# kidusabe1/Imagined-Speech-Decoding

Measured on AMD Instinct MI355X. Metric: trials/sec end-to-end (filterbank+CNN fwd+bwd), higher is better.
Workload: dtype f32; 1 GPU; cfg2: 64ch x 2s@256Hz EEG, 9-band Butterworth(4) filterbank -> STFT(64/32) log band power -> Conv4Layers(576,32)+Linear(32,5) fwd+bwd, softmax-CE, AdamW; trials_per_gpu=4096, global_batch=4096, parallelism=dp1, streams=one stream

## Files before the change

imagined-speech-decoding_amd/csrc/conv.hip:

```cpp
#include "common.h"
#include <math.h>
#include <string.h>
#include <type_traits>
#include <vector>

namespace isd {

typedef float f32x4 __attribute__((ext_vector_type(4)));

constexpr int kTaps = 5;
constexpr int kCK = 32;
constexpr int kMaxZones = 64;

struct ZoneDesc {
  int cin;
  int idx_off;
  int64_t p_off;
  int64_t eff_off;
  int64_t wg_off;
};

struct bf16_t { unsigned short v; };
__device__ __forceinline__ float bf16_round(float x) {
  unsigned int u = __float_as_uint(x);
// ... 1519 lines not shown
    CF_MARK(24);
    __syncthreads();
    CF_MARK(25);
    {
      f32x4 acc[NJ][2];
#pragma unroll
      for (int j = 0; j < NJ; ++j)
#pragma unroll
        for (int gt = 0; gt < 2; ++gt) acc[j][gt] = (f32x4){0.f, 0.f, 0.f, 0.f};
      fused_conv_bf16<NJ>(w3s, gb, ttj, lane, acc);
      fused_store_bf16<NW, false>(acc, nullptr, tA, T1, TT, wave, q, jl);
    }
    CF_MARK(26);
    __syncthreads();
    CF_MARK(27);
    fused_wgrad_bf16(gb_base, tC_base, ct, ks, 4, nkb, q, jl, acc3);
    CF_MARK(28);
    fused_wgrad_x_bf16(tA_base, xt_base, wave, NW, nkb, q, jl, acc0, accb);
    CF_MARK(29);
  }
  {
    float* s4 = a.part4 + ((int64_t)blockIdx.x * 4 + ks) * a.slab1 + (int64_t)z * F * F * kTaps;
    float* s3 = a.part3 + ((int64_t)blockIdx.x * 4 + ks) * a.slab1 + (int64_t)z * F * F * kTaps;
    float* s0 = a.part0 + ((int64_t)blockIdx.x * NW + wave) * a.slab0 + zd.wg_off;
#pragma unroll
    for (int gt = 0; gt < 2; ++gt)
#pragma unroll
      for (int r = 0; r < 4; ++r) {
        const int g = gt * 16 + 4 * q + r, c = ct * 16 + jl;
#pragma unroll
        for (int k = 0; k < kTaps; ++k) {
          s4[((int64_t)g * F + c) * kTaps + k] = acc4[gt][k][r];
          s3[((int64_t)g * F + c) * kTaps + k] = acc3[gt][k][r];
          if (jl < cz) s0[((int64_t)g * cin1 + jl) * kTaps + k] = acc0[gt][k][r];
        }
        if (jl < kTaps) s0[((int64_t)g * cin1 + cz) * kTaps + jl] = jl == 0 ? accb[gt][r] : 0.f;
      }
  }
}

struct TailArgs {
  const void* a2;
  void* g2;
  const float* w3;
  const float* w4;
  const float* w3t;
  const float* w4t;
  const float* fc_w;
  const float* fc_b;
  const void* labels;
  float* logits;
  int64_t* pred;
  float* part;
  int64_t items;
  int T1, n_cls, label_bytes, train, slab;
  float grad_scale;
};

template <int NI>
__device__ __forceinline__ void tail_conv(const float* __restrict__ wl, const float* const (&in)[NI], int T1, int q,
                                          int jl, f32x4 (&acc)[NI][2]) {
  struct Frag {
    float af[kTaps][2];
    float bf[NI][kTaps];
  };
  bool ok[kTaps];
  int off[kTaps];
#pragma unroll
  for (int k = 0; k < kTaps; ++k) {
    const int idx = jl + k - 2;
    ok[k] = idx >= 0 && idx < T1;
    off[k] = ok[k] ? idx : 0;
  }
  auto load = [&](int cg, Frag& f) {
#pragma unroll
    for (int k = 0; k < kTaps; ++k) {
      f.af[k][0] = wl[((cg * kTaps + k) * 2 + 0) * 64];
      f.af[k][1] = wl[((cg * kTaps + k) * 2 + 1) * 64];
#pragma unroll
      for (int i = 0; i < NI; ++i) {
        const float v = in[i][(cg * 4 + q) * T1 + off[k]];
        f.bf[i][k] = ok[k] ? v : 0.f;
      }
    }
  };
  auto mma = [&](const Frag& f) {
#pragma unroll
    for (int k = 0; k < kTaps; ++k)
#pragma unroll
      for (int i = 0; i < NI; ++i) {
        acc[i][0] = __builtin_amdgcn_mfma_f32_16x16x4f32(f.af[k][0], f.bf[i][k], acc[i][0], 0, 0, 0);
        acc[i][1] = __builtin_amdgcn_mfma_f32_16x16x4f32(f.af[k][1], f.bf[i][k], acc[i][1], 0, 0, 0);
      }
  };
  Frag f0, f1;
  load(0, f0);
#pragma unroll 1
  for (int cg = 0; cg < 8; cg += 2) {
    load(cg + 1, f1);
    mma(f0);
    if (cg + 2 < 8) load(cg + 2, f0);
    mma(f1);
  }
}

template <int NI>
__device__ __forceinline__ void tail_wgrad(const float* const (&G)[NI], const float* const (&In)[NI], int T1, int q,
                                           int jl, f32x4 (&acc)[2][2][kTaps]) {
#pragma unroll 1
  for (int s = 0; s < 4; ++s) {
    const int t = s * 4 + q;
    const bool okA = t < T1;
    const int tc = okA ? t : 0;
    float a[NI][2], b[NI][2][kTaps];
#pragma unroll
    for (int i = 0; i < NI; ++i) {
#pragma unroll
      for (int gt = 0; gt < 2; ++gt) {
        const float v = G[i][(gt * 16 + jl) * T1 + tc];
        a[i][gt] = okA ? v : 0.f;
      }
#pragma unroll
      for (int ct = 0; ct < 2; ++ct)
#pragma unroll
        for (int k = 0; k < kTaps; ++k) {
          const int idx = t + k - 2;
          const bool in = okA && idx >= 0 && idx < T1;
          const float v = In[i][(ct * 16 + jl) * T1 + (in ? idx : 0)];
          b[i][ct][k] = in ? v : 0.f;
        }
    }
#pragma unroll
    for (int i = 0; i < NI; ++i)
#pragma unroll
      for (int gt = 0; gt < 2; ++gt)
#pragma unroll
        for (int ct = 0; ct < 2; ++ct)
#pragma unroll
          for (int k = 0; k < kTaps; ++k)
            acc[gt][ct][k] = __builtin_amdgcn_mfma_f32_16x16x4f32(a[i][gt], b[i][ct][k], acc[gt][ct][k], 0, 0, 0);
  }
}

template <bool BF = false>
__device__ __forceinline__ void tail_store_tile(const f32x4 (&acc)[2], float* __restrict__ tile, int T1, int q, int jl) {
  if (jl < T1) {
#pragma unroll
    for (int gt = 0; gt < 2; ++gt)
#pragma unroll
      for (int r = 0; r < 4; ++r) tile[(gt * 16 + 4 * q + r) * T1 + jl] = BF ? bf16_round(acc[gt][r]) : acc[gt][r];
  }
}

constexpr int kTailMaxCls = 16;
constexpr int kTailNI = 1;

constexpr int kTailCombV = 43;
constexpr int kTailCombCopy = kTailCombV * 64 * 4;
template <int NW, int NC, typename WF>
__device__ __forceinline__ void tail_combine_store(float* __restrict__ smem, int wave, int lane, WF&& W,
                                                   const float (&accfc)[kTailMaxCls * 32 / 64], float accb,
                                                   float loss_acc, float* __restrict__ slab, int slab_len, int n_cls) {
  constexpr int F = 32;
  __syncthreads();
  f32x4* mine = reinterpret_cast<f32x4*>(smem + (wave % NC) * kTailCombCopy) + lane;
  constexpr int n_phase = (NW + NC - 1) / NC;
#pragma unroll
  for (int ph = 0; ph < n_phase; ++ph) {
    if (wave / NC == ph) {
      auto put = [&](int v, f32x4 x) {
        if (ph) {
          const f32x4 o = mine[v * 64];
          x[0] += o[0]; x[1] += o[1]; x[2] += o[2]; x[3] += o[3];
        }
        mine[v * 64] = x;
      };
#pragma unroll
      for (int layer = 0; layer < 2; ++layer)
#pragma unroll
        for (int gt = 0; gt < 2; ++gt)
#pragma unroll
          for (int ct = 0; ct < 2; ++ct)
#pragma unroll
            for (int k = 0; k < kTaps; ++k) put(((layer * 2 + gt) * 2 + ct) * kTaps + k, W(layer, gt, ct, k));
      put(40, (f32x4){accfc[0], accfc[1], accfc[2], accfc[3]});
      put(41, (f32x4){accfc[4], accfc[5], accfc[6], accfc[7]});
      put(42, (f32x4){accb, loss_acc, 0.f, 0.f});
    }
    __syncthreads();
  }
  constexpr int n_copy = NW < NC ? NW : NC;
  const int n34 = 2 * F * F * kTaps, o_b = n34 + n_cls * F, o_loss = o_b + n_cls;
  for (int e = threadIdx.x; e < slab_len; e += NW * 64) {
    int src;
    if (e < n34) {
      const int layer = e >= F * F * kTaps, w = e - layer * F * F * kTaps;
      const int g = w / (F * kTaps), rem = w - g * (F * kTaps), c = rem / kTaps, k = rem - c * kTaps;
      const int v = ((layer * 2 + (g >> 4)) * 2 + (c >> 4)) * kTaps + k;
      src = (v * 64 + ((g & 15) >> 2) * 16 + (c & 15)) * 4 + (g & 3);
    } else if (e < o_b) {
      const int f = e - n34, j = f >> 6;
      src = ((40 + (j >> 2)) * 64 + (f & 63)) * 4 + (j & 3);
    } else if (e < o_loss) {
      src = (42 * 64 + (e - o_b)) * 4;
    } else {
      src = (42 * 64) * 4 + 1;
    }
    float v = smem[src];
#pragma unroll
    for (int c = 1; c < n_copy; ++c) v += smem[c * kTailCombCopy + src];
    slab[e] = v;
  }
}

template <int NW, bool BF>
__global__ __launch_bounds__(NW * 64) void featcnn_tail_kernel(TailArgs a) {
  extern __shared__ __attribute__((aligned(16))) float smem[];
  constexpr int F = 32, NI = kTailNI, WF = 8 * kTaps * 2 * 64;
  const int lane = threadIdx.x & 63, wave = threadIdx.x >> 6, q = lane >> 4, jl = lane & 15;
  const int T1 = a.T1, n_cls = a.n_cls;
  const int tile = F * T1, tpad = (tile + 3) & ~3;
  float* w3s = smem;
  float* w4s = w3s + WF;
  float* w3ts = w4s + WF;
  float* w4ts = w3ts + WF;
  float* fcs = w4ts + WF;
  float* priv = fcs + kTailMaxCls * (F + 1) + wave * NI * (4 * tpad + 64);
  float *tA2[NI], *tA3[NI], *tG[NI], *tH[NI], *featL[NI], *logL[NI];
#pragma unroll
  for (int i = 0; i < NI; ++i) {
    float* base = priv + i * (4 * tpad + 64);
    tA2[i] = base;
    tA3[i] = base + tpad;
    tG[i] = base + 2 * tpad;
    tH[i] = base + 3 * tpad;
    featL[i] = base + 4 * tpad;
    logL[i] = featL[i] + 32;
  }
  for (int e = threadIdx.x; e < WF / 4; e += NW * 64) {
    reinterpret_cast<float4*>(w3s)[e] = reinterpret_cast<const float4*>(a.w3)[e];
    reinterpret_cast<float4*>(w4s)[e] = reinterpret_cast<const float4*>(a.w4)[e];
    if (a.train) {
      reinterpret_cast<float4*>(w3ts)[e] = reinterpret_cast<const float4*>(a.w3t)[e];
      reinterpret_cast<float4*>(w4ts)[e] = reinterpret_cast<const float4*>(a.w4t)[e];
    }
  }
  for (int e = threadIdx.x; e < n_cls * F; e += NW * 64) fcs[e] = a.fc_w[e];
  for (int e = threadIdx.x; e < n_cls; e += NW * 64) fcs[n_cls * F + e] = a.fc_b[e];
  __syncthreads();

  f32x4 accW4[2][2][kTaps], accW3[2][2][kTaps];
#pragma unroll
  for (int g = 0; g < 2; ++g)
#pragma unroll
    for (int c = 0; c < 2; ++c)
#pragma unroll
      for (int k = 0; k < kTaps; ++k) {
        accW4[g][c][k] = (f32x4){0.f, 0.f, 0.f, 0.f};
        accW3[g][c][k] = (f32x4){0.f, 0.f, 0.f, 0.f};
      }
  float accfc[kTailMaxCls * F / 64], accb = 0.f, loss_acc = 0.f;
#pragma unroll
  for (int i = 0; i < kTailMaxCls * F / 64; ++i) accfc[i] = 0.f;
  const int n4 = tile >> 2;
  const float inv_t = 1.f / (float)T1;
  const int64_t stride = (int64_t)gridDim.x * NW * NI;

  for (int64_t first = ((int64_t)blockIdx.x * NW + wave) * NI; first < a.items; first += stride) {
    int64_t item[NI];
    bool live[NI];
#pragma unroll
    for (int i = 0; i < NI; ++i) {
      live[i] = first + i < a.items;
      item[i] = live[i] ? first + i : first;
      if constexpr (BF) {
        if (lane < 4 * T1) {
          const uint4 w = reinterpret_cast<const uint4*>((const unsigned short*)a.a2 + item[i] * tile)[lane];
          const int t = lane >> 2, g0 = (lane & 3) * 8;
          float* d = tA2[i] + g0 * T1 + t;
          d[0] = bf16_lo(w.x); d[T1] = bf16_hi(w.x); d[2 * T1] = bf16_lo(w.y); d[3 * T1] = bf16_hi(w.y);
          d[4 * T1] = bf16_lo(w.z); d[5 * T1] = bf16_hi(w.z); d[6 * T1] = bf16_lo(w.w); d[7 * T1] = bf16_hi(w.w);
        }
      } else {
        const float4* src = reinterpret_cast<const float4*>((const float*)a.a2 + item[i] * tile);
        float4* dst = reinterpret_cast<float4*>(tA2[i]);
        if (lane < n4) dst[lane] = src[lane];
        if (lane + 64 < n4) dst[lane + 64] = src[lane + 64];
      }
    }
    wave_lds_sync();
    f32x4 acc[NI][2];
    auto clear = [&]() {
#pragma unroll
      for (int i = 0; i < NI; ++i) {
        acc[i][0] = (f32x4){0.f, 0.f, 0.f, 0.f};
        acc[i][1] = (f32x4){0.f, 0.f, 0.f, 0.f};
      }
    };
    clear();
    tail_conv<NI>(w3s + lane, tA2, T1, q, jl, acc);
#pragma unroll
    for (int i = 0; i < NI; ++i) tail_store_tile<BF>(acc[i], tA3[i], T1, q, jl);
    wave_lds_sync();
    clear();
    tail_conv<NI>(w4s + lane, tA3, T1, q, jl, acc);
    if constexpr (BF) {
#pragma unroll
      for (int i = 0; i < NI; ++i)
#pragma unroll
        for (int gt = 0; gt < 2; ++gt)
#pragma unroll
          for (int r = 0; r < 4; ++r) acc[i][gt][r] = bf16_round(acc[i][gt][r]);
    }
#pragma unroll
    for (int i = 0; i < NI; ++i)
#pragma unroll
      for (int gt = 0; gt < 2; ++gt)
#pragma unroll
        for (int r = 0; r < 4; ++r) {
          float sacc = jl < T1 ? gelu_f(acc[i][gt][r]) : 0.f;
          sacc += row_shr<8>(sacc);
          sacc += row_shr<4>(sacc);
          sacc += row_shr<2>(sacc);
          sacc += row_shr<1>(sacc);
          if (jl == 15) featL[i][gt * 16 + 4 * q + r] = sacc * inv_t;
        }
    wave_lds_sync();
#pragma unroll
    for (int i = 0; i < NI; ++i)
      if (lane < n_cls) {
        float l = fcs[n_cls * F + lane];
#pragma unroll
        for (int g = 0; g < F; ++g) l = fmaf(fcs[lane * F + g], featL[i][g], l);
        logL[i][lane] = l;
        if (live[i]) a.logits[item[i] * n_cls + lane] = l;
      }
    wave_lds_sync();
    float lse[NI];
    int yv[NI];
#pragma unroll
    for (int i = 0; i < NI; ++i) {
      float mx = -INFINITY;
      int am = 0;
      for (int c = 0; c < n_cls; ++c) {
        const float v = logL[i][c];
        if (v > mx) { mx = v; am = c; }
      }
      if (lane == 0 && live[i]) a.pred[item[i]] = am;
      lse[i] = 0.f;
      yv[i] = 0;
      if (a.labels) {
        float se = 0.f;
        for (int c = 0; c < n_cls; ++c) se += expf(logL[i][c] - mx);
        yv[i] = a.label_bytes == 1 ? (int)((const unsigned char*)a.labels)[item[i]]
                                   : (int)((const long long*)a.labels)[item[i]];
        lse[i] = mx + logf(se);
        if (lane == 0 && live[i]) loss_acc += (lse[i] - logL[i][yv[i]]) * a.grad_scale;
      }
    }
    if (!a.labels || !a.train) continue;
#pragma unroll
    for (int i = 0; i < NI; ++i)
      if (lane < n_cls)
        logL[i][16 + lane] = live[i] ? (expf(logL[i][lane] - lse[i]) - (lane == yv[i] ? 1.f : 0.f)) * a.grad_scale : 0.f;
    wave_lds_sync();
#pragma unroll
    for (int i = 0; i < NI; ++i) {
#pragma unroll
      for (int gt = 0; gt < 2; ++gt)
#pragma unroll
        for (int r = 0; r < 4; ++r) {
          const int g = gt * 16 + 4 * q + r;
          float d = 0.f;
          for (int c = 0; c < n_cls; ++c) d = fmaf(fcs[c * F + g], logL[i][16 + c], d);
          acc[i][gt][r] = d * inv_t * gelu_grad_f(acc[i][gt][r]);
        }
      tail_store_tile<BF>(acc[i], tG[i], T1, q, jl);
#pragma unroll
      for (int j = 0; j < kTailMaxCls * F / 64; ++j) {
        const int e = lane + 64 * j;
        if (e < n_cls * F) accfc[j] = fmaf(logL[i][16 + (e >> 5)], featL[i][e & 31], accfc[j]);
      }
      if (lane < n_cls) accb += logL[i][16 + lane];
    }
    wave_lds_sync();
    tail_wgrad<NI>(tG, tA3, T1, q, jl, accW4);
    clear();
    tail_conv<NI>(w4ts + lane, tG, T1, q, jl, acc);
#pragma unroll
    for (int i = 0; i < NI; ++i) tail_store_tile<BF>(acc[i], tH[i], T1, q, jl);
    wave_lds_sync();
    tail_wgrad<NI>(tH, tA2, T1, q, jl, accW3);
    clear();
    tail_conv<NI>(w3ts + lane, tH, T1, q, jl, acc);
    wave_lds_sync();
#pragma unroll
    for (int i = 0; i < NI; ++i) tail_store_tile(acc[i], tG[i], T1, q, jl);
    wave_lds_sync();
#pragma unroll
    for (int i = 0; i < NI; ++i)
      if (live[i]) {
        if constexpr (BF) {
          if (lane < 4 * T1) {
            const int t = lane >> 2, g0 = (lane & 3) * 8;
            const float* sp = tG[i] + g0 * T1 + t;
            uint4 w;
            w.x = bf16_pack(sp[0], sp[T1]); w.y = bf16_pack(sp[2 * T1], sp[3 * T1]);
            w.z = bf16_pack(sp[4 * T1], sp[5 * T1]); w.w = bf16_pack(sp[6 * T1], sp[7 * T1]);
            reinterpret_cast<uint4*>((unsigned short*)a.g2 + item[i] * tile)[lane] = w;
          }
        } else {
          float4* dst = reinterpret_cast<float4*>((float*)a.g2 + item[i] * tile);
          const float4* src = reinterpret_cast<const float4*>(tG[i]);
          if (lane < n4) dst[lane] = src[lane];
          if (lane + 64 < n4) dst[lane + 64] = src[lane + 64];
        }
      }
    wave_lds_sync();
  }
  if (!a.labels) return;
  tail_combine_store<NW, 2>(smem, wave, lane,
                            [&](int layer, int gt, int ct, int k) -> f32x4 { return layer ? accW4[gt][ct][k] : accW3[gt][ct][k]; },
                            accfc, accb, loss_acc, a.part + (int64_t)blockIdx.x * a.slab, a.slab, n_cls);
}

template <int NW>
__global__ __launch_bounds__(NW * 64) void featcnn_tail_bf16_kernel(TailArgs a) {
  extern __shared__ __attribute__((aligned(16))) float smem[];
  constexpr int F = 32, FR = kTaps * 2 * 64;
  constexpr int R = 40, tile_b = R * 64;
  constexpr int priv_b = 4 * tile_b + 256;
  const int lane = threadIdx.x & 63, wave = threadIdx.x >> 6, q = lane >> 4, jl = lane & 15;
  const int T1 = a.T1, n_cls = a.n_cls;
  uint4* w3s = reinterpret_cast<uint4*>(smem);
  uint4* w4s = w3s + FR;
  uint4* w3ts = w4s + FR;
  uint4* w4ts = w3ts + FR;
  float* fcs = reinterpret_cast<float*>(w4ts + FR);
  char* priv = reinterpret_cast<char*>(fcs + kTailMaxCls * (F + 1)) + wave * priv_b;
  char* tA2 = priv;
  char* tA3 = priv + tile_b;
  char* tG = priv + 2 * tile_b;
  char* tH = priv + 3 * tile_b;
  float* featL = reinterpret_cast<float*>(priv + 4 * tile_b);
  float* logL = featL + 32;
  const unsigned smem_base = (unsigned)(uintptr_t)(__attribute__((address_space(3))) float*)smem;
  const unsigned priv_base = smem_base + (unsigned)(4 * FR * 16 + kTailMaxCls * (F + 1) * 4 + wave * priv_b);
  for (int e = threadIdx.x; e < FR; e += NW * 64) {
    w3s[e] = reinterpret_cast<const uint4*>(a.w3)[e];
    w4s[e] = reinterpret_cast<const uint4*>(a.w4)[e];
    if (a.train) {
      w3ts[e] = reinterpret_cast<const uint4*>(a.w3t)[e];
      w4ts[e] = reinterpret_cast<const uint4*>(a.w4t)[e];
    }
  }
  for (int e = threadIdx.x; e < n_cls * F; e += NW * 64) fcs[e] = a.fc_w[e];
  for (int e = threadIdx.x; e < n_cls; e += NW * 64) fcs[n_cls * F + e] = a.fc_b[e];
  for (int e = lane; e < priv_b / 16; e += 64) reinterpret_cast<uint4*>(priv)[e] = make_uint4(0u, 0u, 0u, 0u);
  __syncthreads();

  f32x4 accW4[2][2][kTaps], accW3[2][2][kTaps];
#pragma unroll
  for (int c = 0; c < 2; ++c)
#pragma unroll
    for (int g = 0; g < 2; ++g)
#pragma unroll
      for (int k = 0; k < kTaps; ++k) {
        accW4[c][g][k] = (f32x4){0.f, 0.f, 0.f, 0.f};
        accW3[c][g][k] = (f32x4){0.f, 0.f, 0.f, 0.f};
      }
  float accfc[kTailMaxCls * F / 64], accb = 0.f, loss_acc = 0.f;
#pragma unroll
  for (int i = 0; i < kTailMaxCls * F / 64; ++i) accfc[i] = 0.f;
  const int tile = F * T1;
  const float inv_t = 1.f / (float)T1;
// ... 52 lines not shown
    wave_lds_sync();
    float mx = -INFINITY, lse = 0.f;
    int am = 0, yv = 0;
    for (int c = 0; c < n_cls; ++c) {
      const float v = logL[c];
      if (v > mx) { mx = v; am = c; }
    }
    if (lane == 0 && live) a.pred[item] = am;
    if (a.labels) {
      float se = 0.f;
      for (int c = 0; c < n_cls; ++c) se += expf(logL[c] - mx);
      yv = a.label_bytes == 1 ? (int)((const unsigned char*)a.labels)[item] : (int)((const long long*)a.labels)[item];
      lse = mx + logf(se);
      if (lane == 0 && live) loss_acc += (lse - logL[yv]) * a.grad_scale;
    }
    if (!a.labels || !a.train) continue;
    if (lane < n_cls) logL[16 + lane] = live ? (expf(logL[lane] - lse) - (lane == yv ? 1.f : 0.f)) * a.grad_scale : 0.f;
    wave_lds_sync();
#pragma unroll
    for (int gt = 0; gt < 2; ++gt)
#pragma unroll
      for (int r = 0; r < 4; ++r) {
        const int g = gt * 16 + 4 * q + r;
        float d = 0.f;
        for (int c = 0; c < n_cls; ++c) d = fmaf(fcs[c * F + g], logL[16 + c], d);
        acc[0][gt][r] = d * inv_t * gelu_grad_f(acc[0][gt][r]);
      }
    store_tile(acc[0], tG);
#pragma unroll
    for (int j = 0; j < kTailMaxCls * F / 64; ++j) {
      const int e = lane + 64 * j;
      if (e < n_cls * F) accfc[j] = fmaf(logL[16 + (e >> 5)], featL[e & 31], accfc[j]);
    }
    if (lane < n_cls) accb += logL[16 + lane];
    wave_lds_sync();
    fused_wgrad_bf16(priv_base + 2 * tile_b, priv_base + tile_b, 0, 0, 1, 1, q, jl, accW4[0]);
    fused_wgrad_bf16(priv_base + 2 * tile_b, priv_base + tile_b, 1, 0, 1, 1, q, jl, accW4[1]);
    clear();
    fused_conv_bf16<1>(w4ts, tG, tt0, lane, acc);
    store_tile(acc[0], tH);
    wave_lds_sync();
    fused_wgrad_bf16(priv_base + 3 * tile_b, priv_base, 0, 0, 1, 1, q, jl, accW3[0]);
    fused_wgrad_bf16(priv_base + 3 * tile_b, priv_base, 1, 0, 1, 1, q, jl, accW3[1]);
    clear();
    fused_conv_bf16<1>(w3ts, tH, tt0, lane, acc);
    wave_lds_sync();
    store_tile(acc[0], tG);
    wave_lds_sync();
    if (live && lane < 4 * T1)
      reinterpret_cast<uint4*>((unsigned short*)a.g2 + item * tile)[lane] = *reinterpret_cast<const uint4*>(tG + 128 + lane * 16);
    wave_lds_sync();
  }
  if (!a.labels) return;
  tail_combine_store<NW, 3>(smem, wave, lane,
                            [&](int layer, int gt, int ct, int k) -> f32x4 { return layer ? accW4[ct][gt][k] : accW3[ct][gt][k]; },
                            accfc, accb, loss_acc, a.part + (int64_t)blockIdx.x * a.slab, a.slab, n_cls);
}

template <typename AT>
__global__ __launch_bounds__(256) void gelu_mean_fwd_kernel(const void* __restrict__ a, float* __restrict__ feat,
                                                            int64_t rows, int T) {
  const int64_t row = ((int64_t)blockIdx.x * 256 + threadIdx.x) >> 4;
  const int i = threadIdx.x & 15;
  float s = 0.f;
  if (row < rows) {
    for (int t = i; t < T; t += 16) s += gelu_f(Act<AT>::ld(a, row * T + t));
  }
  s += row_shr<8>(s);
  s += row_shr<4>(s);
  s += row_shr<2>(s);
  s += row_shr<1>(s);
  if (row < rows && i == 15) feat[row] = s / (float)T;
}

template <typename AT, bool PRE = false>
__global__ __launch_bounds__(256) void gelu_mean_bwd_kernel(void* __restrict__ a, const float* __restrict__ dfeat,
                                                            int64_t rows, int T) {
  const int64_t row = ((int64_t)blockIdx.x * 256 + threadIdx.x) >> 4;
  const int i = threadIdx.x & 15;
  if (row >= rows) return;
  const float g = dfeat[row] / (float)T;
  for (int t = i; t < T; t += 16) {
    const float v = Act<AT>::ld(a, row * T + t);
    Act<AT>::st(a, row * T + t, g * (PRE ? v : gelu_grad_f(v)));
  }
}

__global__ __launch_bounds__(256) void conv5_dx_kernel(const float* __restrict__ g2, const float* __restrict__ wfrag,
                                                       const ZoneDesc* __restrict__ zones,
                                                       const int* __restrict__ chan_idx, float* __restrict__ dx,
                                                       int Z, int F, int T1, int W, int Ctot, int Tx, int N, int S) {
  extern __shared__ __attribute__((aligned(16))) float smem[];
  const int64_t item = blockIdx.x;
  const int z = blockIdx.y;
  const ZoneDesc zd = zones[z];
  const int GT = F / 16;
  const float* src = g2 + (item * Z + z) * (int64_t)(F * T1);
  for (int e = threadIdx.x; e < F * T1; e += 256) smem[e] = src[e];
  __syncthreads();
  const int64_t b = item / N;
  const int n = (int)(item - b * N);
  const float* wz = wfrag + zd.eff_off;
  for (int e = threadIdx.x; e < zd.cin * W; e += 256) {
    const int c = e / W, t = e - c * W;
    const int cg = c >> 2, cl = (c & 3) * 16;
    float acc = 0.f;
    for (int g = 0; g < F; ++g) {
// ... 742 lines not shown
  for (int z = 0; z < n_zones; ++z)
    for (int c = 1; c < zone_sizes[z]; ++c)
      if (idx[zd[z].idx_off + c] != idx[zd[z].idx_off + c - 1] + 1) p->contiguous = 0;
  p->dma_ok = p->contiguous && (c_total % 4 == 0);
  for (int z = 0; z < n_zones; ++z)
    if (zone_sizes[z] % 4 != 0 || idx[zd[z].idx_off] % 4 != 0) p->dma_ok = 0;
  p->conv_zstride = (int64_t)(F / 4) * kTaps * GT * 64;
  hipError_t e = hipMalloc(&p->d_zones, sizeof(ZoneDesc) * n_zones);
  if (e == hipSuccess) e = hipMalloc(&p->d_idx, sizeof(int) * idx.size());
  if (e == hipSuccess) e = hipMemcpy(p->d_zones, zd.data(), sizeof(ZoneDesc) * n_zones, hipMemcpyHostToDevice);
  if (e == hipSuccess) e = hipMemcpy(p->d_idx, idx.data(), sizeof(int) * idx.size(), hipMemcpyHostToDevice);
  if (e != hipSuccess) {
    set_error("isd_conv4_plan_create: %s", hipGetErrorString(e));
    isd_conv4_plan_destroy(p);
    return e == hipErrorNoDevice ? ISD_ERR_NO_DEVICE : ISD_ERR_HIP;
  }
  *out = p;
  return ISD_OK;
}

extern "C" int isd_conv4_plan_destroy(isd_conv4_plan* p) {
  if (!p) return ISD_OK;
  if (p->d_zones) (void)hipFree(p->d_zones);
  if (p->d_idx) (void)hipFree(p->d_idx);
  delete p;
  return ISD_OK;
}

extern "C" int isd_conv4_plan_set_activation_dtype(isd_conv4_plan* p, int dtype) {
  ISD_CHECK_ARG(p && (dtype == ISD_ACT_F32 || dtype == ISD_ACT_BF16), "isd_conv4_plan_set_activation_dtype: bad argument");
  p->act_bf16 = dtype == ISD_ACT_BF16;
  return ISD_OK;
}

extern "C" int64_t isd_conv4_param_count(const isd_conv4_plan* p) { return p ? p->n_params : ISD_ERR_INVALID; }

extern "C" int64_t isd_conv4_param_offset(const isd_conv4_plan* p, int zone, int which) {
  if (!p || zone < 0 || zone >= p->Z || which < 0 || which > 4 || (which > 2 && p->n_layers != 4)) return ISD_ERR_INVALID;
  const int64_t F = p->F;
  const int64_t offs[5] = {0, F * kTaps, F * kTaps + F, F * kTaps + F + F * F * p->cz[zone],
                           F * kTaps + F + F * F * p->cz[zone] + F * F * kTaps};
  return p->p_off[zone] + offs[which];
}

extern "C" int isd_conv4_windows(const isd_conv4_plan* p, int64_t T) {
  if (!p || T < p->W) return ISD_ERR_INVALID;
  return (int)((T - p->W) / p->S + 1);
}

namespace {
struct Geo {
  int N, T1, TT, IPW, RS_a, RS_b, lin0, CK;
  int64_t items, act;
  int64_t o_eff, o_eff16, o_beff, o_w3, o_w3t, o_w4, o_w4t, o_a2, o_a3, o_a4, o_s, o_wg, o_wg34, o_part, total;
  int ipw0, ipw1, ns0, ns1, cw0, cw1, grp0, grp1;
  int64_t slab0, slab1;
};

int row_stride_fwd(int need) {
  if (need <= 32) return need | 1;
  int rs = need;
  while (rs % 32 != 16) ++rs;
  return rs;
}

int make_geo(const isd_conv4_plan* p, int64_t B, int64_t T, Geo& g) {
  ISD_CHECK_ARG(T >= p->W, "conv4: T=%lld shorter than window_len=%d", (long long)T, p->W);
  g.N = (int)((T - p->W) / p->S + 1);
  g.T1 = p->W - (kTaps - 1);
  g.TT = (g.T1 + 15) / 16;
  g.IPW = g.TT >= 16 ? 1 : 16 / g.TT;
  g.items = B * g.N;
  g.act = g.items * p->Z * p->F * g.T1;
  g.lin0 = (p->contiguous && g.N == 1 && T == p->W) ? 1 : 0;
  g.RS_a = g.lin0 ? p->W : row_stride_fwd(p->W);
  g.RS_b = g.T1;
  {
    const int GTf = p->F / 16;
    const int64_t row = g.RS_a > g.RS_b ? g.RS_a : g.RS_b;
    g.CK = kCK;
    int64_t fit = (64 * 1024 / 4 - (int64_t)(g.CK / 4) * kTaps * GTf * 64) / (g.CK * row);
    if (fit < 1) {
      while (g.CK > 4 && (150 * 1024 / 4 - 64 - (int64_t)(g.CK / 4) * kTaps * GTf * 64) / (g.CK * row) < 1) g.CK -= 4;
      fit = (150 * 1024 / 4 - 64 - (int64_t)(g.CK / 4) * kTaps * GTf * 64) / (g.CK * row);
    }
    ISD_CHECK_ARG(fit >= 1, "conv4: window_len=%d is too long for the LDS tile (about 9000 samples)", p->W);
    if (g.IPW > fit) g.IPW = (int)fit;
    const int64_t occ = (g.items * p->Z) / 512;
    int min_ipw = (4 + g.TT - 1) / g.TT;
    if (min_ipw < 1) min_ipw = 1;
    int64_t want = occ < min_ipw ? min_ipw : occ;
    if (g.IPW > want) g.IPW = (int)want;
  }
  int64_t o = 0;
  g.o_eff = o;  o += align_up(p->eff_size, 64);
  g.o_eff16 = o; o += align_up(p->eff_size / kTaps * 4, 64);
  g.o_beff = o; o += align_up((int64_t)p->Z * p->F, 64);
  const int64_t cw = align_up(p->conv_zstride * p->Z, 64);
  g.o_w3 = o; o += cw; g.o_w3t = o; o += cw; g.o_w4 = o; o += cw; g.o_w4t = o; o += cw;
  g.o_a2 = o; o += align_up(g.act, 64);
  g.o_a3 = o; o += align_up(g.act, 64);
  g.o_a4 = o; o += align_up(g.act, 64);
  g.o_s = o;  o += align_up(g.act, 64);
  g.o_wg = o; o += align_up(p->wg_size, 64);
  g.slab1 = (int64_t)p->Z * p->F * p->F * kTaps;
  g.o_wg34 = o; o += align_up(g.slab1, 64);
  const int GT = p->F / 16;
  auto plan_wg = [&](int cin_max, int& cw, int& ipw, int& ns, int& grp) {
    cw = cin_max >= 64 ? 64 : (int)align_up(cin_max, 16);
    grp = 4 / (cw / 16);
    const int zg = (cin_max + cw - 1) / cw;
    int64_t want = 1024 / ((int64_t)p->Z * zg);
    if (want < 1) want = 1;
    const int64_t it = g.items > 0 ? g.items : 1;
    if (want > it) want = it;
    ipw = (int)cdiv(it, want);
    ns = (int)cdiv(it, ipw) * grp;
  };
  plan_wg(p->max_cz + 1, g.cw0, g.ipw0, g.ns0, g.grp0);
  plan_wg(p->F, g.cw1, g.ipw1, g.ns1, g.grp1);
  g.slab0 = p->wg_size;
  const int64_t pa = (int64_t)g.ns0 * g.slab0, pb = (p->n_layers == 4) ? (int64_t)g.ns1 * g.slab1 : 0;
  const int64_t rz = 256 / p->Z > 1 ? 256 / p->Z : 1;
  const int64_t pf = (p->n_layers == 4) ? rz * (8 * g.slab1 + 8 * g.slab0) : 0;
  const int64_t pmax = pa > pb ? pa : pb;
  g.o_part = o; o += align_up(pmax > pf ? pmax : pf, 64);
  g.total = o;
  return ISD_OK;
}
}

extern "C" int64_t isd_conv4_workspace_bytes(const isd_conv4_plan* p, int64_t B, int64_t T) {
  if (!p || B < 0) return ISD_ERR_INVALID;
  Geo g;
  if (make_geo(p, B, T, g)) return ISD_ERR_INVALID;
  return g.total * 4;
}

static int launch_conv(int mode, int bf16, const ConvArgs& a, int n_zones, hipStream_t st) {
  const int64_t blocks = cdiv(a.items, a.IPW);
  ISD_CHECK_ARG(blocks <= 0x7fffffffLL, "conv4: too many items");
  const int GT = a.F / 16;
  const size_t lds = sizeof(float) * (4 + (((size_t)a.IPW * a.CK * a.RS + 3) & ~(size_t)3) + (size_t)(a.CK / 4) * kTaps * GT * 64 + 32);
  ISD_CHECK_ARG(lds <= 150 * 1024, "conv4: LDS tile of %zu bytes exceeds 150 KiB (window too long)", lds);
  const dim3 grid((unsigned)blocks, n_zones);
  const int tiles = a.IPW * a.TT;
  const int NT = tiles > 8 ? 4 : tiles > 4 ? 2 : 1;
#define ISD_CONV_LAUNCH_1(M, T, G, N)                                                                \
  do {                                                                                               \
    if (lds > 48 * 1024)                                                                             \
      ISD_HIP_TRY(hipFuncSetAttribute((const void*)conv5_fwd_kernel<M, T, G, N>,                     \
                                      hipFuncAttributeMaxDynamicSharedMemorySize, (int)lds));        \
    hipLaunchKernelGGL((conv5_fwd_kernel<M, T, G, N>), grid, dim3(256), lds, st, a);                 \
  } while (0)
#define ISD_CONV_LAUNCH_N(M, T, G)                                                                   \
  do {                                                                                               \
// ... 328 lines not shown
  return ISD_OK;
}

static bool featcnn_ok(const isd_conv4_plan* p, const Geo& g, int n_cls, const void* x = nullptr) {
  return p->Z == 1 && p->n_layers == 4 && p->F == 32 && (!p->act_bf16 || bf16_mfma_ok(p, g, x)) && g.TT == 1 &&
         g.N == 1 && n_cls >= 1 && n_cls <= kTailMaxCls;
}

extern "C" int isd_featcnn_supported(const isd_conv4_plan* p, int64_t B, int64_t T, int n_cls) {
  if (!p || B < 1) return 0;
  Geo g;
  if (make_geo(p, B, T, g)) return 0;
  return featcnn_ok(p, g, n_cls) ? 1 : 0;
}

static int featcnn_step_impl(const isd_conv4_plan* p, const float* x, const float* params, const float* fc_w,
                             const float* fc_b, const void* labels, int label_bytes, float* dparams, float* dfc,
                             float* logits, int64_t* pred, float* loss, void* workspace, int64_t B, int64_t T,
                             int n_cls, float grad_scale, void* stream, bool x_bf16) {
  ISD_CHECK_ARG(p, "isd_featcnn_step: null plan");
  ISD_CHECK_ARG(B >= 1, "isd_featcnn_step: B=%lld", (long long)B);
  Geo g;
  int rc = make_geo(p, B, T, g);
  if (rc) return rc;
  if (!featcnn_ok(p, g, n_cls, x)) {
    set_error("isd_featcnn_step: needs one zone, 4 layers, 32 filters, <= 16 output steps (bf16 activations: <= 13, over "
              "whole 16-byte aligned rows of at most 17 samples), <= %d classes", kTailMaxCls);
    return ISD_ERR_UNSUPPORTED;
  }
  const bool tap16 = p->act_bf16 != 0;
  if (x_bf16 && !(tap16 && p->max_cz % 8 == 0)) {
    set_error("isd_featcnn_step_bf16: a bf16 feature map needs a plan with bf16 activations and a multiple of 8 input "
              "channels (got act_bf16=%d, %d channels)", p->act_bf16, p->max_cz);
    return ISD_ERR_UNSUPPORTED;
  }
  ISD_CHECK_ARG(x && params && fc_w && fc_b && logits && pred && workspace, "isd_featcnn_step: null argument");
  ISD_CHECK_ARG(!labels || label_bytes == 1 || label_bytes == 8, "isd_featcnn_step: labels must be uint8 or int64");
  const bool train = labels && dparams && dfc;
  ISD_CHECK_ARG(!labels || loss, "isd_featcnn_step: labels without a loss pointer");
  hipStream_t st = (hipStream_t)stream;
  float* ws = (float*)workspace;
  const int F = p->F;
  rc = launch_prep(p, g, params, ws, st, tap16);
  if (rc) return rc;
  ConvArgs a = {};
  rc = first_layer_forward(p, g, x, T, ws, st, a, tap16, x_bf16);
  if (rc) return rc;
  TailArgs t = {};
  t.a2 = ws + g.o_a2; t.g2 = ws + g.o_a4;
  t.w3 = ws + g.o_w3; t.w4 = ws + g.o_w4; t.w3t = ws + g.o_w3t; t.w4t = ws + g.o_w4t;
  t.fc_w = fc_w; t.fc_b = fc_b; t.labels = labels; t.label_bytes = label_bytes;
  t.logits = logits; t.pred = pred; t.part = ws + g.o_part;
  t.items = g.items; t.T1 = g.T1; t.n_cls = n_cls; t.train = train ? 1 : 0; t.grad_scale = grad_scale;
  const int n34 = 2 * F * F * kTaps, nfc = n_cls * (F + 1);
  t.slab = n34 + nfc + 1;
  constexpr int TNW = 4;
  int blocks = (int)cdiv(g.items, TNW * kTailNI * 2);
  if (blocks > 256) blocks = 256;
  if (blocks < 1) blocks = 1;
  const int tile = (F * g.T1 + 3) & ~3;
  size_t lds = sizeof(float) * (size_t)(4 * 8 * kTaps * 2 * 64 + kTailMaxCls * (F + 1) + TNW * kTailNI * (4 * tile + 64) + 16);
  if (lds < sizeof(float) * 2 * kTailCombCopy) lds = sizeof(float) * 2 * kTailCombCopy;
  ISD_CHECK_ARG(lds <= 160 * 1024 && (int64_t)blocks * t.slab <= g.total - g.o_part, "isd_featcnn_step: workspace");
  if (tap16) {
    constexpr int BNW = 8;
    blocks = (int)cdiv(g.items, BNW * 2);
    if (blocks > 256) blocks = 256;
    if (blocks < 1) blocks = 1;
    size_t lds16 = (size_t)4 * kTaps * 2 * 64 * 16 + sizeof(float) * kTailMaxCls * (F + 1) + (size_t)BNW * (4 * 40 * 64 + 256) + 64;
    if (lds16 < sizeof(float) * 3 * kTailCombCopy) lds16 = sizeof(float) * 3 * kTailCombCopy;
    ISD_CHECK_ARG(lds16 <= 160 * 1024 && (int64_t)blocks * t.slab <= g.total - g.o_part, "isd_featcnn_step: workspace");
    ISD_HIP_TRY(hipFuncSetAttribute((const void*)featcnn_tail_bf16_kernel<BNW>, hipFuncAttributeMaxDynamicSharedMemorySize, (int)lds16));
    hipLaunchKernelGGL((featcnn_tail_bf16_kernel<BNW>), dim3(blocks), dim3(BNW * 64), lds16, st, t);
  } else {
    ISD_HIP_TRY(hipFuncSetAttribute((const void*)featcnn_tail_kernel<TNW, false>, hipFuncAttributeMaxDynamicSharedMemorySize, (int)lds));
    hipLaunchKernelGGL((featcnn_tail_kernel<TNW, false>), dim3(blocks), dim3(TNW * 64), lds, st, t);
  }
  ISD_LAUNCH_CHECK();
  if (!labels) return ISD_OK;
  if (train) {
    float* dw34 = dparams + p->p_off[0] + F * kTaps + F + (int64_t)F * F * p->cz[0];
    launch_reduce_slabs(ws + g.o_part, ReduceDst{dw34, dfc, loss, n34, nfc}, t.slab, blocks, st);
  } else {
    float* red = ws + g.o_s;
    launch_reduce_slabs(ws + g.o_part, ReduceDst{red, red + n34, loss, n34, nfc}, t.slab, blocks, st);
  }
  ISD_LAUNCH_CHECK();
  if (!train) return ISD_OK;
  return first_layer_backward(p, g, x, T, params, ws + g.o_a4, dparams, ws, st, tap16, x_bf16);
}

extern "C" int isd_featcnn_step(const isd_conv4_plan* p, const float* x, const float* params, const float* fc_w,
                                const float* fc_b, const void* labels, int label_bytes, float* dparams, float* dfc,
                                float* logits, int64_t* pred, float* loss, void* workspace, int64_t B, int64_t T,
                                int n_cls, float grad_scale, void* stream) {
  return featcnn_step_impl(p, x, params, fc_w, fc_b, labels, label_bytes, dparams, dfc, logits, pred, loss, workspace, B,
                           T, n_cls, grad_scale, stream, false);
}

extern "C" int isd_featcnn_step_bf16(const isd_conv4_plan* p, const uint16_t* x, const float* params, const float* fc_w,
                                     const float* fc_b, const void* labels, int label_bytes, float* dparams, float* dfc,
                                     float* logits, int64_t* pred, float* loss, void* workspace, int64_t B, int64_t T,
                                     int n_cls, float grad_scale, void* stream) {
  return featcnn_step_impl(p, reinterpret_cast<const float*>(x), params, fc_w, fc_b, labels, label_bytes, dparams, dfc,
                           logits, pred, loss, workspace, B, T, n_cls, grad_scale, stream, true);
}

static int conv4_backward_impl(const isd_conv4_plan* p, const float* x, const float* params, const float* dfeat,
                               float* dparams, float* dx, void* workspace, int64_t B, int64_t T, void* stream) {
  ISD_CHECK_ARG(p, "isd_conv4_backward: null plan");
// ... 152 lines not shown
```

Measured before the change: 3.570 million trials/s.

## Split tail weight-gradient accumulation into a separate per-block pass over spilled tiles

The fp32 tail kernel no longer keeps both conv3 and conv4 weight-gradient MFMA accumulators live in every wave during the per-item loop. Instead each wave writes its A3, G4 and G3 tiles plus features, logit gradients and loss to global scratch. A second phase reloads them in batches into LDS and lets dedicated waves accumulate either the W4 or the W3 gradient. Waves per block double to 8 to cut register pressure and raise occupancy, at the cost of extra global writes and reads for the spilled tiles and new workspace buffers.

After: 3.596 million trials/s, median of 6. About the same (+0.7%).

```diff
diff --git a/imagined-speech-decoding_amd/csrc/conv.hip b/imagined-speech-decoding_amd/csrc/conv.hip
--- a/imagined-speech-decoding_amd/csrc/conv.hip
+++ b/imagined-speech-decoding_amd/csrc/conv.hip
@@ -1595,6 +1595,10 @@
   float* logits;
   int64_t* pred;
   float* part;
+  float* a3;
+  float* g4;
+  float* g3;
+  float* ts;
   int64_t items;
   int T1, n_cls, label_bytes, train, slab;
   float grad_scale;
@@ -1696,12 +1700,13 @@
 }
 
 constexpr int kTailMaxCls = 16;
+constexpr int kTailAccW = 4;
 constexpr int kTailNI = 1;
 
 constexpr int kTailCombV = 43;
 constexpr int kTailCombCopy = kTailCombV * 64 * 4;
-template <int NW, int NC, typename WF>
-__device__ __forceinline__ void tail_combine_store(float* __restrict__ smem, int wave, int lane, WF&& W,
+template <int NW, int NC, int NT, typename WF>
+__device__ __forceinline__ void tail_combine_store(float* __restrict__ smem, int wave, int own, int lane, WF&& W,
                                                    const float (&accfc)[kTailMaxCls * 32 / 64], float accb,
                                                    float loss_acc, float* __restrict__ slab, int slab_len, int n_cls) {
   constexpr int F = 32;
@@ -1720,21 +1725,25 @@
       };
 #pragma unroll
       for (int layer = 0; layer < 2; ++layer)
-#pragma unroll
-        for (int gt = 0; gt < 2; ++gt)
-#pragma unroll
-          for (int ct = 0; ct < 2; ++ct)
-#pragma unroll
-            for (int k = 0; k < kTaps; ++k) put(((layer * 2 + gt) * 2 + ct) * kTaps + k, W(layer, gt, ct, k));
-      put(40, (f32x4){accfc[0], accfc[1], accfc[2], accfc[3]});
-      put(41, (f32x4){accfc[4], accfc[5], accfc[6], accfc[7]});
-      put(42, (f32x4){accb, loss_acc, 0.f, 0.f});
+        if (own >> layer & 1) {
+#pragma unroll
+          for (int gt = 0; gt < 2; ++gt)
+#pragma unroll
+            for (int ct = 0; ct < 2; ++ct)
+#pragma unroll
+              for (int k = 0; k < kTaps; ++k) put(((layer * 2 + gt) * 2 + ct) * kTaps + k, W(layer, gt, ct, k));
+        }
+      if (own & 4) {
+        put(40, (f32x4){accfc[0], accfc[1], accfc[2], accfc[3]});
+        put(41, (f32x4){accfc[4], accfc[5], accfc[6], accfc[7]});
+        put(42, (f32x4){accb, loss_acc, 0.f, 0.f});
+      }
     }
     __syncthreads();
   }
   constexpr int n_copy = NW < NC ? NW : NC;
   const int n34 = 2 * F * F * kTaps, o_b = n34 + n_cls * F, o_loss = o_b + n_cls;
-  for (int e = threadIdx.x; e < slab_len; e += NW * 64) {
+  for (int e = threadIdx.x; e < slab_len; e += NT) {
     int src;
     if (e < n34) {
       const int layer = e >= F * F * kTaps, w = e - layer * F * F * kTaps;
@@ -1769,6 +1778,11 @@
   float* w4ts = w3ts + WF;
   float* fcs = w4ts + WF;
   float* priv = fcs + kTailMaxCls * (F + 1) + wave * NI * (4 * tpad + 64);
+  const int n4 = tile >> 2;
+  auto tile_copy = [&](const float* __restrict__ src, float* __restrict__ dst) {
+    if (lane < n4) reinterpret_cast<float4*>(dst)[lane] = reinterpret_cast<const float4*>(src)[lane];
+    if (lane + 64 < n4) reinterpret_cast<float4*>(dst)[lane + 64] = reinterpret_cast<const float4*>(src)[lane + 64];
+  };
   float *tA2[NI], *tA3[NI], *tG[NI], *tH[NI], *featL[NI], *logL[NI];
 #pragma unroll
   for (int i = 0; i < NI; ++i) {
@@ -1780,6 +1794,19 @@
     featL[i] = base + 4 * tpad;
     logL[i] = featL[i] + 32;
   }
+  auto load_a2 = [&](int64_t item, float* __restrict__ dst) {
+    if constexpr (BF) {
+      if (lane < 4 * T1) {
+        const uint4 w = reinterpret_cast<const uint4*>((const unsigned short*)a.a2 + item * tile)[lane];
+        const int t = lane >> 2, g0 = (lane & 3) * 8;
+        float* d = dst + g0 * T1 + t;
+        d[0] = bf16_lo(w.x); d[T1] = bf16_hi(w.x); d[2 * T1] = bf16_lo(w.y); d[3 * T1] = bf16_hi(w.y);
+        d[4 * T1] = bf16_lo(w.z); d[5 * T1] = bf16_hi(w.z); d[6 * T1] = bf16_lo(w.w); d[7 * T1] = bf16_hi(w.w);
+      }
+    } else {
+      tile_copy((const float*)a.a2 + item * tile, dst);
+    }
+  };
   for (int e = threadIdx.x; e < WF / 4; e += NW * 64) {
     reinterpret_cast<float4*>(w3s)[e] = reinterpret_cast<const float4*>(a.w3)[e];
     reinterpret_cast<float4*>(w4s)[e] = reinterpret_cast<const float4*>(a.w4)[e];
@@ -1792,44 +1819,23 @@
   for (int e = threadIdx.x; e < n_cls; e += NW * 64) fcs[n_cls * F + e] = a.fc_b[e];
   __syncthreads();
 
-  f32x4 accW4[2][2][kTaps], accW3[2][2][kTaps];
-#pragma unroll
-  for (int g = 0; g < 2; ++g)
-#pragma unroll
-    for (int c = 0; c < 2; ++c)
-#pragma unroll
-      for (int k = 0; k < kTaps; ++k) {
-        accW4[g][c][k] = (f32x4){0.f, 0.f, 0.f, 0.f};
-        accW3[g][c][k] = (f32x4){0.f, 0.f, 0.f, 0.f};
-      }
   float accfc[kTailMaxCls * F / 64], accb = 0.f, loss_acc = 0.f;
 #pragma unroll
   for (int i = 0; i < kTailMaxCls * F / 64; ++i) accfc[i] = 0.f;
-  const int n4 = tile >> 2;
   const float inv_t = 1.f / (float)T1;
-  const int64_t stride = (int64_t)gridDim.x * NW * NI;
-
-  for (int64_t first = ((int64_t)blockIdx.x * NW + wave) * NI; first < a.items; first += stride) {
+  static_assert(NI == 1, "one item per wave and step");
+  const int64_t acc_stride = (int64_t)gridDim.x * kTailAccW;
+  auto blk_item = [&](int j) -> int64_t {
+    return (int64_t)blockIdx.x * kTailAccW + j % kTailAccW + (int64_t)(j / kTailAccW) * acc_stride;
+  };
+  for (int j = wave; blk_item(j) < a.items; j += NW) {
     int64_t item[NI];
     bool live[NI];
 #pragma unroll
     for (int i = 0; i < NI; ++i) {
-      live[i] = first + i < a.items;
-      item[i] = live[i] ? first + i : first;
-      if constexpr (BF) {
-        if (lane < 4 * T1) {
-          const uint4 w = reinterpret_cast<const uint4*>((const unsigned short*)a.a2 + item[i] * tile)[lane];
-          const int t = lane >> 2, g0 = (lane & 3) * 8;
-          float* d = tA2[i] + g0 * T1 + t;
-          d[0] = bf16_lo(w.x); d[T1] = bf16_hi(w.x); d[2 * T1] = bf16_lo(w.y); d[3 * T1] = bf16_hi(w.y);
-          d[4 * T1] = bf16_lo(w.z); d[5 * T1] = bf16_hi(w.z); d[6 * T1] = bf16_lo(w.w); d[7 * T1] = bf16_hi(w.w);
-        }
-      } else {
-        const float4* src = reinterpret_cast<const float4*>((const float*)a.a2 + item[i] * tile);
-        float4* dst = reinterpret_cast<float4*>(tA2[i]);
-        if (lane < n4) dst[lane] = src[lane];
-        if (lane + 64 < n4) dst[lane + 64] = src[lane + 64];
-      }
+      live[i] = true;
+      item[i] = blk_item(j);
+      load_a2(item[i], tA2[i]);
     }
     wave_lds_sync();
     f32x4 acc[NI][2];
@@ -1898,7 +1904,7 @@
         yv[i] = a.label_bytes == 1 ? (int)((const unsigned char*)a.labels)[item[i]]
                                    : (int)((const long long*)a.labels)[item[i]];
         lse[i] = mx + logf(se);
-        if (lane == 0 && live[i]) loss_acc += (lse[i] - logL[i][yv[i]]) * a.grad_scale;
+        if (lane == 0) a.ts[item[i] * 64 + 48] = lse[i] - logL[i][yv[i]];
       }
     }
     if (!a.labels || !a.train) continue;
@@ -1919,21 +1925,24 @@
           acc[i][gt][r] = d * inv_t * gelu_grad_f(acc[i][gt][r]);
         }
       tail_store_tile<BF>(acc[i], tG[i], T1, q, jl);
-#pragma unroll
-      for (int j = 0; j < kTailMaxCls * F / 64; ++j) {
-        const int e = lane + 64 * j;
-        if (e < n_cls * F) accfc[j] = fmaf(logL[i][16 + (e >> 5)], featL[i][e & 31], accfc[j]);
-      }
-      if (lane < n_cls) accb += logL[i][16 + lane];
+      if (lane < F) a.ts[item[i] * 64 + lane] = featL[i][lane];
+      if (lane < n_cls) a.ts[item[i] * 64 + 32 + lane] = logL[i][16 + lane];
     }
     wave_lds_sync();
-    tail_wgrad<NI>(tG, tA3, T1, q, jl, accW4);
+#pragma unroll
+    for (int i = 0; i < NI; ++i)
+      if (live[i]) {
+        tile_copy(tA3[i], a.a3 + item[i] * tile);
+        tile_copy(tG[i], a.g4 + item[i] * tile);
+      }
     clear();
     tail_conv<NI>(w4ts + lane, tG, T1, q, jl, acc);
 #pragma unroll
     for (int i = 0; i < NI; ++i) tail_store_tile<BF>(acc[i], tH[i], T1, q, jl);
     wave_lds_sync();
-    tail_wgrad<NI>(tH, tA2, T1, q, jl, accW3);
+#pragma unroll
+    for (int i = 0; i < NI; ++i)
+      if (live[i]) tile_copy(tH[i], a.g3 + item[i] * tile);
     clear();
     tail_conv<NI>(w3ts + lane, tH, T1, q, jl, acc);
     wave_lds_sync();
@@ -1953,17 +1962,86 @@
             reinterpret_cast<uint4*>((unsigned short*)a.g2 + item[i] * tile)[lane] = w;
           }
         } else {
-          float4* dst = reinterpret_cast<float4*>((float*)a.g2 + item[i] * tile);
-          const float4* src = reinterpret_cast<const float4*>(tG[i]);
-          if (lane < n4) dst[lane] = src[lane];
-          if (lane + 64 < n4) dst[lane + 64] = src[lane + 64];
+          tile_copy(tG[i], (float*)a.g2 + item[i] * tile);
         }
       }
     wave_lds_sync();
   }
   if (!a.labels) return;
-  tail_combine_store<NW, 2>(smem, wave, lane,
-                            [&](int layer, int gt, int ct, int k) -> f32x4 { return layer ? accW4[gt][ct][k] : accW3[gt][ct][k]; },
+  static_assert(!BF, "the accumulation pass reads A2 as fp32");
+  f32x4 accW[2][2][kTaps];
+#pragma unroll
+  for (int g = 0; g < 2; ++g)
+#pragma unroll
+    for (int c = 0; c < 2; ++c)
+#pragma unroll
+      for (int k = 0; k < kTaps; ++k) accW[g][c][k] = (f32x4){0.f, 0.f, 0.f, 0.f};
+  const int SL = 4 * tpad + 64;
+  const int rounds = (4 * WF + kTailMaxCls * (F + 1) + NW * NI * (4 * tpad + 64)) / SL / kTailAccW;
+  const int per = a.train ? 4 * n4 + 16 : 16;
+  static_assert(NW == 2 * kTailAccW, "two waves per sum slot");
+  const int sw = wave % kTailAccW, own = wave < kTailAccW ? 6 : 1;
+  int n_blk = 0;
+  while (blk_item(n_blk) < a.items) ++n_blk;
+  __syncthreads();
+  for (int j0 = 0; j0 < n_blk; j0 += rounds * kTailAccW) {
+    const int j1 = j0 + rounds * kTailAccW < n_blk ? j0 + rounds * kTailAccW : n_blk;
+    constexpr int U = 8;
+    const int n_st = (j1 - j0) * per;
+    for (int e0 = threadIdx.x; e0 < n_st; e0 += U * NW * 64) {
+      float4 r[U];
+      int d[U];
+#pragma unroll
+      for (int uu = 0; uu < U; ++uu) {
+        const int e = e0 + uu * NW * 64;
+        d[uu] = -1;
+        r[uu] = (float4){0.f, 0.f, 0.f, 0.f};
+        if (e < n_st) {
+          const int sl = e / per, u = e - sl * per;
+          const int64_t it = blk_item(j0 + sl);
+          if (u >= per - 16) {
+            d[uu] = (sl * SL + 4 * tpad) / 4 + (u - (per - 16));
+            r[uu] = reinterpret_cast<const float4*>(a.ts + it * 64)[u - (per - 16)];
+          } else {
+            const int t = u / n4, v = u - t * n4;
+            const float* src = t == 0 ? (const float*)a.a2 : t == 1 ? a.a3 : t == 2 ? a.g4 : a.g3;
+            d[uu] = (sl * SL + t * tpad) / 4 + v;
+            r[uu] = reinterpret_cast<const float4*>(src + it * tile)[v];
+          }
+        }
+      }
+#pragma unroll
+      for (int uu = 0; uu < U; ++uu)
+        if (d[uu] >= 0) reinterpret_cast<float4*>(smem)[d[uu]] = r[uu];
+    }
+    __syncthreads();
+    for (int j = j0 + sw; j < j1; j += kTailAccW) {
+      const float* slot = smem + (j - j0) * SL;
+      const float* sc = slot + 4 * tpad;
+      if (own & 4) {
+        if (lane == 0) loss_acc += sc[48] * a.grad_scale;
+        if (a.train) {
+#pragma unroll
+          for (int i = 0; i < kTailMaxCls * F / 64; ++i) {
+            const int e = lane + 64 * i;
+            if (e < n_cls * F) accfc[i] = fmaf(sc[32 + (e >> 5)], sc[e & 31], accfc[i]);
+          }
+          if (lane < n_cls) accb += sc[32 + lane];
+        }
+      }
+      if (a.train) {
+        const float* const sA2[1] = {slot};
+        const float* const sA3[1] = {slot + tpad};
+        const float* const sG4[1] = {slot + 2 * tpad};
+        const float* const sG3[1] = {slot + 3 * tpad};
+        if (own & 2) tail_wgrad<1>(sG4, sA3, T1, q, jl, accW);
+        else tail_wgrad<1>(sG3, sA2, T1, q, jl, accW);
+      }
+    }
+    __syncthreads();
+  }
+  tail_combine_store<kTailAccW, 2, NW * 64>(smem, sw, own, lane,
+                            [&](int, int gt, int ct, int k) -> f32x4 { return accW[gt][ct][k]; },
                             accfc, accb, loss_acc, a.part + (int64_t)blockIdx.x * a.slab, a.slab, n_cls);
 }
 
@@ -2122,7 +2200,7 @@
     wave_lds_sync();
   }
   if (!a.labels) return;
-  tail_combine_store<NW, 3>(smem, wave, lane,
+  tail_combine_store<NW, 3, NW * 64>(smem, wave, 7, lane,
                             [&](int layer, int gt, int ct, int k) -> f32x4 { return layer ? accW4[ct][gt][k] : accW3[ct][gt][k]; },
                             accfc, accb, loss_acc, a.part + (int64_t)blockIdx.x * a.slab, a.slab, n_cls);
 }
@@ -2971,7 +3049,7 @@
 struct Geo {
   int N, T1, TT, IPW, RS_a, RS_b, lin0, CK;
   int64_t items, act;
-  int64_t o_eff, o_eff16, o_beff, o_w3, o_w3t, o_w4, o_w4t, o_a2, o_a3, o_a4, o_s, o_wg, o_wg34, o_part, total;
+  int64_t o_eff, o_eff16, o_beff, o_w3, o_w3t, o_w4, o_w4t, o_a2, o_a3, o_a4, o_s, o_g3, o_ts, o_wg, o_wg34, o_part, total;
   int ipw0, ipw1, ns0, ns1, cw0, cw1, grp0, grp1;
   int64_t slab0, slab1;
 };
@@ -3021,6 +3099,8 @@
   g.o_a3 = o; o += align_up(g.act, 64);
   g.o_a4 = o; o += align_up(g.act, 64);
   g.o_s = o;  o += align_up(g.act, 64);
+  g.o_g3 = o; o += align_up(g.act, 64);
+  g.o_ts = o; o += align_up(g.items * 64, 64);
   g.o_wg = o; o += align_up(p->wg_size, 64);
   g.slab1 = (int64_t)p->Z * p->F * p->F * kTaps;
   g.o_wg34 = o; o += align_up(g.slab1, 64);
@@ -3455,10 +3535,11 @@
   t.fc_w = fc_w; t.fc_b = fc_b; t.labels = labels; t.label_bytes = label_bytes;
   t.logits = logits; t.pred = pred; t.part = ws + g.o_part;
   t.items = g.items; t.T1 = g.T1; t.n_cls = n_cls; t.train = train ? 1 : 0; t.grad_scale = grad_scale;
+  t.a3 = ws + g.o_a3; t.g4 = ws + g.o_s; t.g3 = ws + g.o_g3; t.ts = ws + g.o_ts;
   const int n34 = 2 * F * F * kTaps, nfc = n_cls * (F + 1);
   t.slab = n34 + nfc + 1;
-  constexpr int TNW = 4;
-  int blocks = (int)cdiv(g.items, TNW * kTailNI * 2);
+  constexpr int TNW = 8;
+  int blocks = (int)cdiv(g.items, kTailAccW * 2);
   if (blocks > 256) blocks = 256;
   if (blocks < 1) blocks = 1;
   const int tile = (F * g.T1 + 3) & ~3;
```
